# whwu95/MVFNet

Measured on AMD Instinct MI355X. Metric: clips/sec (fwd+bwd) MVFNet-R50 8x8 224^2, higher is better.
Workload: dtype bf16; 1 GPU; MVFNet-ResNet50 8x8, 32 clips/GPU of 8x3x224x224, bf16, train step: fwd (batch-stat BN) + loss + bwd + clip + SGD-nesterov; all through the HIP C ABI (stem + 16 bottlenecks + MVF + TSN head); clips_per_gpu=32, frames_per_clip=8, parallelism=dp1: replicas, one flat gradient all-reduce per step

## Files before the change

### mvfnet_amd/csrc/bn_dzfree.hip

```cpp
#include "common.h"

namespace {

typedef float f32x16 __attribute__((ext_vector_type(16)));
typedef short bf16x8 __attribute__((ext_vector_type(8)));

struct PrepArgs {
    const uint16_t* wd;
    const float *gamma, *mean, *invstd, *dgamma, *dbeta;
    uint16_t* bd;
    float* bias;
    int C, K;
    float inv_m;
    int g_wgs, s_wgs;
};

__device__ __forceinline__ float bf16lo(unsigned u) { return __uint_as_float(u << 16); }
__device__ __forceinline__ float bf16hi(unsigned u) { return __uint_as_float(u & 0xffff0000u); }

__global__ __launch_bounds__(256) void dzfree_prep_kernel(PrepArgs p) {
    extern __shared__ __attribute__((aligned(16))) float coef[];
    const int C = p.C, K = p.K, tid = threadIdx.x;
    float* ca = coef;
    float* ce = coef + C;
    float* ct = coef + 2 * C;
    for (int c = tid; c < C; c += 256) {
        const float r = p.invstd[c], a = p.gamma[c] * r, d0 = p.dbeta[c] * p.inv_m, kx = r * p.dgamma[c] * p.inv_m;
        ca[c] = a;
        ce[c] = a * kx;
        ct[c] = a * (d0 - kx * p.mean[c]);
    }
    __syncthreads();
    const int lane = tid & 63, wave = tid >> 6;
    int b = blockIdx.x;
    if (b < p.g_wgs) {
        const int kb = K / 32;
        const int j0 = (b / kb) * 32, k0 = (b % kb) * 32;
        const int row = lane & 31, half = lane >> 5;
        const int cq = C / 4, cbeg = wave * cq;
        const uint16_t* pa = p.wd + (long)(j0 + row) * C + half * 8;
        const uint16_t* pb = p.wd + (long)(k0 + row) * C + half * 8;
        f32x16 acc;
#pragma unroll
        for (int r = 0; r < 16; ++r) acc[r] = 0.f;
        uint4 va[4], vb[4], na[4], nb[4];
#pragma unroll
        for (int s_ = 0; s_ < 4; ++s_) {
            va[s_] = *reinterpret_cast<const uint4*>(pa + cbeg + s_ * 16);
            vb[s_] = *reinterpret_cast<const uint4*>(pb + cbeg + s_ * 16);
        }
        for (int c0 = cbeg; c0 < cbeg + cq; c0 += 64) {
            const bool more = c0 + 64 < cbeg + cq;
#pragma unroll
            for (int s_ = 0; s_ < 4; ++s_) {
                na[s_] = more ? *reinterpret_cast<const uint4*>(pa + c0 + 64 + s_ * 16) : make_uint4(0, 0, 0, 0);
                nb[s_] = more ? *reinterpret_cast<const uint4*>(pb + c0 + 64 + s_ * 16) : make_uint4(0, 0, 0, 0);
            }
#pragma unroll
            for (int s_ = 0; s_ < 4; ++s_) {
                const float4 e0 = *reinterpret_cast<const float4*>(ce + c0 + s_ * 16 + half * 8), e1 = *reinterpret_cast<const float4*>(ce + c0 + s_ * 16 + half * 8 + 4);
                uint4 sa;
                sa.x = pack_bf16x2(bf16lo(va[s_].x) * e0.x, bf16hi(va[s_].x) * e0.y);
                sa.y = pack_bf16x2(bf16lo(va[s_].y) * e0.z, bf16hi(va[s_].y) * e0.w);
                sa.z = pack_bf16x2(bf16lo(va[s_].z) * e1.x, bf16hi(va[s_].z) * e1.y);
                sa.w = pack_bf16x2(bf16lo(va[s_].w) * e1.z, bf16hi(va[s_].w) * e1.w);
                bf16x8 fa, fb;
                __builtin_memcpy(&fa, &sa, 16);
                __builtin_memcpy(&fb, &vb[s_], 16);
                acc = __builtin_amdgcn_mfma_f32_32x32x16_bf16(fa, fb, acc, 0, 0, 0);
            }
#pragma unroll
            for (int s_ = 0; s_ < 4; ++s_) { va[s_] = na[s_]; vb[s_] = nb[s_]; }
        }
        float* red = coef + 3 * C;
#pragma unroll
        for (int r = 0; r < 16; ++r) red[(wave * 16 + r) * 64 + lane] = acc[r];
        __syncthreads();
        float v[4];
#pragma unroll
        for (int i = 0; i < 4; ++i) v[i] = (red[(0 * 16 + 4 * wave + i) * 64 + lane] + red[(1 * 16 + 4 * wave + i) * 64 + lane]) +
                                           (red[(2 * 16 + 4 * wave + i) * 64 + lane] + red[(3 * 16 + 4 * wave + i) * 64 + lane]);
        uint2 pk;
        pk.x = pack_bf16x2(-v[0], -v[1]);
        pk.y = pack_bf16x2(-v[2], -v[3]);
        *reinterpret_cast<uint2*>(p.bd + (long)(k0 + row) * (C + K) + C + j0 + 4 * half + 8 * wave) = pk;
        return;
    }
    b -= p.g_wgs;
    if (b < p.s_wgs) {
        const long u = (long)b * 256 + tid, per_row = C / 8;
        if (u >= (long)K * per_row) return;
        const int k = (int)(u / per_row), c = (int)(u - (long)k * per_row) * 8;
        const uint4 v = *reinterpret_cast<const uint4*>(p.wd + (long)k * C + c);
        const float4 a0 = *reinterpret_cast<const float4*>(ca + c), a1 = *reinterpret_cast<const float4*>(ca + c + 4);
        uint4 o;
        o.x = pack_bf16x2(bf16lo(v.x) * a0.x, bf16hi(v.x) * a0.y);
        o.y = pack_bf16x2(bf16lo(v.y) * a0.z, bf16hi(v.y) * a0.w);
        o.z = pack_bf16x2(bf16lo(v.z) * a1.x, bf16hi(v.z) * a1.y);
        o.w = pack_bf16x2(bf16lo(v.w) * a1.z, bf16hi(v.w) * a1.w);
        *reinterpret_cast<uint4*>(p.bd + (long)k * (C + K) + c) = o;
        return;
    }
    b -= p.s_wgs;
    {
        const int k = b * 4 + wave;
        if (k >= K) return;
        float s = 0.f;
        for (int c = lane * 8; c < C; c += 512) {
            const uint4 v = *reinterpret_cast<const uint4*>(p.wd + (long)k * C + c);
            const float4 t0 = *reinterpret_cast<const float4*>(ct + c), t1 = *reinterpret_cast<const float4*>(ct + c + 4);
            s += bf16lo(v.x) * t0.x + bf16hi(v.x) * t0.y + bf16lo(v.y) * t0.z + bf16hi(v.y) * t0.w;
            s += bf16lo(v.z) * t1.x + bf16hi(v.z) * t1.y + bf16lo(v.w) * t1.z + bf16hi(v.w) * t1.w;
        }
        for (int off = 32; off >= 1; off >>= 1) s += __shfl_xor(s, off, 64);
        if (lane == 0) p.bias[k] = -s;
    }
}

__global__ __launch_bounds__(256) void dzfree_wgrad_fix_kernel(float* dw, const uint16_t* w, const float* gram, const float* a_mean, const float* gamma,
                                                               const float* mean, const float* invstd, const float* dgamma, const float* dbeta, int C, int K,
                                                               float m_f) {
    const int lane = threadIdx.x & 63, wave = threadIdx.x >> 6;
    const int kb = K / 32, blk = blockIdx.x * 4 + wave;
    if (blk >= (C / 32) * kb) return;
    const int c0 = (blk / kb) * 32, k0 = (blk % kb) * 32;
    const int row = lane & 31, half = lane >> 5;
    const uint16_t* pw = w + (long)(c0 + row) * K + half * 8;
    const float* pg = gram + (long)(k0 + row) * K + half * 8;
    f32x16 acc;
#pragma unroll
    for (int r = 0; r < 16; ++r) acc[r] = 0.f;
    constexpr int U = 4;
    for (int j = 0; j < K; j += 16 * U) {
        uint4 vw[U];
        float4 g0[U], g1[U];
#pragma unroll
        for (int u = 0; u < U; ++u) {
            vw[u] = *reinterpret_cast<const uint4*>(pw + j + 16 * u);
            g0[u] = *reinterpret_cast<const float4*>(pg + j + 16 * u);
            g1[u] = *reinterpret_cast<const float4*>(pg + j + 16 * u + 4);
        }
#pragma unroll
        for (int u = 0; u < U; ++u) {
            uint4 hi, lo;
            hi.x = pack_bf16x2(g0[u].x, g0[u].y); hi.y = pack_bf16x2(g0[u].z, g0[u].w);
            hi.z = pack_bf16x2(g1[u].x, g1[u].y); hi.w = pack_bf16x2(g1[u].z, g1[u].w);
            lo.x = pack_bf16x2(g0[u].x - bf16lo(hi.x), g0[u].y - bf16hi(hi.x)); lo.y = pack_bf16x2(g0[u].z - bf16lo(hi.y), g0[u].w - bf16hi(hi.y));
            lo.z = pack_bf16x2(g1[u].x - bf16lo(hi.z), g1[u].y - bf16hi(hi.z)); lo.w = pack_bf16x2(g1[u].z - bf16lo(hi.w), g1[u].w - bf16hi(hi.w));
            bf16x8 fw, fh, fl;
            __builtin_memcpy(&fw, &vw[u], 16);
            __builtin_memcpy(&fh, &hi, 16);
            __builtin_memcpy(&fl, &lo, 16);
            acc = __builtin_amdgcn_mfma_f32_32x32x16_bf16(fw, fh, acc, 0, 0, 0);
            acc = __builtin_amdgcn_mfma_f32_32x32x16_bf16(fw, fl, acc, 0, 0, 0);
        }
    }
    const float inv_m = 1.0f / m_f;
    const int k = k0 + row;
    const float sa = a_mean[k] * m_f;
#pragma unroll
    for (int r = 0; r < 16; ++r) {
        const int c = c0 + 8 * (r >> 2) + 4 * half + (r & 3);
        const float rs = invstd[c], a = gamma[c] * rs, d0 = dbeta[c] * inv_m, kx = rs * dgamma[c] * inv_m;
        const long i = (long)c * K + k;
        dw[i] = a * (dw[i] - d0 * sa - kx * (acc[r] - mean[c] * sa));
    }
}

__global__ __launch_bounds__(256) void dzfree_sums_kernel(const float* q, const uint16_t* w, int C, int K, const float* mean,
                                                          const float* invstd, const float* part_lo, int rows_lo, int c_split, const float* part_hi, int rows_hi,
                                                          float* dgamma, float* dbeta) {
    const int lane = threadIdx.x & 63, c = blockIdx.x * 4 + (threadIdx.x >> 6);
    if (c >= C) return;
    const bool lo = c < c_split;
    const int rows = lo ? rows_lo : rows_hi;
    const float2* p = reinterpret_cast<const float2*>(lo ? part_lo : part_hi) + (long)c * rows;
    float s1 = 0.f, dot = 0.f;
    for (int r = lane; r < rows; r += 64) s1 += p[r].x;
    const uint16_t* pw = w + (long)c * K;
    const float* pq = q + (long)c * K;
    for (int k = lane * 4; k < K; k += 256) {
        const uint2 wv = *reinterpret_cast<const uint2*>(pw + k);
        const float4 qv = *reinterpret_cast<const float4*>(pq + k);
        dot += bf16lo(wv.x) * qv.x + bf16hi(wv.x) * qv.y + bf16lo(wv.y) * qv.z + bf16hi(wv.y) * qv.w;
    }
#pragma unroll
    for (int o = 32; o > 0; o >>= 1) {
        s1 += __shfl_xor(s1, o, 64);
        dot += __shfl_xor(dot, o, 64);
    }
    if (lane == 0) {
        dbeta[c] = s1;
        dgamma[c] = invstd[c] * (dot - mean[c] * s1);
    }
}

struct GramStatsArgs {
    const float* gram; const float* a_mean; const uint16_t* w; const float* gamma; const float* beta;
    float* running_mean; float* running_var; float* save_mean; float* save_invstd; float* scale; float* shift;
    int C, K; float inv_m, eps, momentum, unbias;
};
__global__ __launch_bounds__(256) void gram_stats_kernel(GramStatsArgs p) {
    const int lane = threadIdx.x & 63, wave = threadIdx.x >> 6, K = p.K;
    const int blk = blockIdx.x * 4 + wave;
    if (blk >= p.C / 32) return;
    const int c0 = blk * 32, row = lane & 31, half = lane >> 5;
    const uint16_t* pw = p.w + (long)(c0 + row) * K + half * 8;
    float qacc[16], macc[16];
#pragma unroll
    for (int r = 0; r < 16; ++r) qacc[r] = macc[r] = 0.f;
    for (int kb = 0; kb < K / 32; ++kb) {
        const int k = kb * 32 + row;
        const float* pg = p.gram + (long)k * K + half * 8;
        const float* pa = p.a_mean + half * 8;
        const float ak = p.a_mean[k];
        f32x16 acc;
#pragma unroll
        for (int r = 0; r < 16; ++r) acc[r] = 0.f;
        for (int j = 0; j < K; j += 16) {
            const uint4 vw = *reinterpret_cast<const uint4*>(pw + j);
            const float4 g0 = *reinterpret_cast<const float4*>(pg + j), g1 = *reinterpret_cast<const float4*>(pg + j + 4);
            const float4 a0 = *reinterpret_cast<const float4*>(pa + j), a1 = *reinterpret_cast<const float4*>(pa + j + 4);
            float gc[8] = {g0.x * p.inv_m - ak * a0.x, g0.y * p.inv_m - ak * a0.y, g0.z * p.inv_m - ak * a0.z, g0.w * p.inv_m - ak * a0.w,
                           g1.x * p.inv_m - ak * a1.x, g1.y * p.inv_m - ak * a1.y, g1.z * p.inv_m - ak * a1.z, g1.w * p.inv_m - ak * a1.w};
            unsigned hi[4], mid[4], lo[4];
#pragma unroll
            for (int q = 0; q < 4; ++q) {
                const float x0 = gc[2 * q], x1 = gc[2 * q + 1];
                hi[q] = pack_bf16x2(x0, x1);
                const float r0 = x0 - bf16lo(hi[q]), r1 = x1 - bf16hi(hi[q]);
                mid[q] = pack_bf16x2(r0, r1);
                lo[q] = pack_bf16x2(r0 - bf16lo(mid[q]), r1 - bf16hi(mid[q]));
            }
            bf16x8 fw, fh, fm, fl;
            __builtin_memcpy(&fw, &vw, 16);
            __builtin_memcpy(&fh, hi, 16);
            __builtin_memcpy(&fm, mid, 16);
            __builtin_memcpy(&fl, lo, 16);
            acc = __builtin_amdgcn_mfma_f32_32x32x16_bf16(fw, fh, acc, 0, 0, 0);
            acc = __builtin_amdgcn_mfma_f32_32x32x16_bf16(fw, fm, acc, 0, 0, 0);
            acc = __builtin_amdgcn_mfma_f32_32x32x16_bf16(fw, fl, acc, 0, 0, 0);
        }
#pragma unroll
        for (int r = 0; r < 16; ++r) {
            const int c = c0 + 8 * (r >> 2) + 4 * half + (r & 3);
            const float wv = __uint_as_float((unsigned)p.w[(long)c * K + k] << 16);
            qacc[r] += acc[r] * wv;
            macc[r] += wv * ak;
        }
    }
#pragma unroll
    for (int r = 0; r < 16; ++r) {
#pragma unroll
        for (int o = 1; o < 32; o <<= 1) {
            qacc[r] += __shfl_xor(qacc[r], o, 64);
            macc[r] += __shfl_xor(macc[r], o, 64);
        }
    }
    if (row == 0) {
#pragma unroll
        for (int r = 0; r < 16; ++r) {
            const int c = c0 + 8 * (r >> 2) + 4 * half + (r & 3);
            const float mean = macc[r], var = fmaxf(qacc[r], 0.f);
            const float invstd = 1.0f / sqrtf(var + p.eps);
            p.save_mean[c] = mean;
            p.save_invstd[c] = invstd;
            const float s = p.gamma[c] * invstd;
            p.scale[c] = s;
            p.shift[c] = p.beta[c] - mean * s;
            if (p.running_mean) p.running_mean[c] = (1.f - p.momentum) * p.running_mean[c] + p.momentum * mean;
            if (p.running_var) p.running_var[c] = (1.f - p.momentum) * p.running_var[c] + p.momentum * (var * p.unbias);
        }
    }
}

}

extern "C" {

int mvf_bn_train_stats_gram(const float* gram, const float* a_mean, const void* w_packed, long m, int c, int k, const float* gamma, const float* beta, float eps,
                            float momentum, float* running_mean, float* running_var, float* save_mean, float* save_invstd, float* scale, float* shift,
                            int dtype, void* stream) {
    MVF_REQUIRE(gram && a_mean && w_packed && gamma && beta && save_mean && save_invstd && scale && shift && m > 0, MVF_EINVAL, "bn_train_stats_gram: NULL argument");
    MVF_REQUIRE(dtype == MVF_BF16, MVF_EUNSUPPORTED, "bn_train_stats_gram: bf16 storage only");
    MVF_REQUIRE(c > 0 && k > 0 && c % 32 == 0 && k % 32 == 0, MVF_ESHAPE, "bn_train_stats_gram: c=%d and k=%d must be multiples of 32", c, k);
    MVF_REQUIRE(((uintptr_t)gram | (uintptr_t)a_mean | (uintptr_t)w_packed) % 16 == 0, MVF_EINVAL, "bn_train_stats_gram: operands must be 16-byte aligned");
    GramStatsArgs p = {gram, a_mean, (const uint16_t*)w_packed, gamma, beta, running_mean, running_var, save_mean, save_invstd, scale, shift,
                       c, k, 1.0f / (float)m, eps, momentum, (float)((double)m / (double)(m > 1 ? m - 1 : 1))};
    hipLaunchKernelGGL(gram_stats_kernel, dim3((c / 32 + 3) / 4), dim3(256), 0, (hipStream_t)stream, p);
    MVF_LAUNCH_CHECK();
    return MVF_OK;
}

int mvf_bn_bwd_dzfree_sums(const float* q, const void* w_packed, int c, int k, const float* mean, const float* invstd,
                           const float* part_lo, int rows_lo, int c_split, const float* part_hi, int rows_hi, float* dgamma, float* dbeta, int dtype, void* stream) {
    MVF_REQUIRE(q && w_packed && mean && invstd && dgamma && dbeta, MVF_EINVAL, "bn_bwd_dzfree_sums: NULL argument");
    MVF_REQUIRE(dtype == MVF_BF16, MVF_EUNSUPPORTED, "bn_bwd_dzfree_sums: bf16 storage only");
    MVF_REQUIRE(c > 0 && k > 0 && k % 4 == 0 && c_split >= 0 && c_split <= c, MVF_ESHAPE, "bn_bwd_dzfree_sums: c=%d, k=%d (a multiple of 4), 0 <= c_split=%d <= c", c, k, c_split);
    MVF_REQUIRE((c_split == 0 || (part_lo && rows_lo > 0)) && (c_split == c || (part_hi && rows_hi > 0)), MVF_EINVAL, "bn_bwd_dzfree_sums: a channel range without partial sums");
    MVF_REQUIRE(((uintptr_t)q % 16 == 0) && ((uintptr_t)w_packed % 8 == 0), MVF_EINVAL, "bn_bwd_dzfree_sums: q must be 16-byte, w_packed 8-byte aligned");
    hipLaunchKernelGGL(dzfree_sums_kernel, dim3((c + 3) / 4), dim3(256), 0, (hipStream_t)stream, q, (const uint16_t*)w_packed, c, k, mean, invstd, part_lo, rows_lo,
                       c_split, part_hi, rows_hi, dgamma, dbeta);
    MVF_LAUNCH_CHECK();
    return MVF_OK;
}

int mvf_bn_bwd_dzfree_prep(const void* w_packed_dgrad, int c, int k, const float* gamma, const float* mean, const float* invstd, const float* dgamma,
                           const float* dbeta, long m, void* w_out, float* bias_out, int dtype, void* stream) {
    MVF_REQUIRE(w_packed_dgrad && gamma && mean && invstd && dgamma && dbeta && w_out && bias_out && m > 0, MVF_EINVAL, "bn_bwd_dzfree_prep: NULL argument");
    MVF_REQUIRE(dtype == MVF_BF16, MVF_EUNSUPPORTED, "bn_bwd_dzfree_prep: bf16 storage only");
    MVF_REQUIRE(c > 0 && k > 0 && c % 64 == 0 && k % 32 == 0 && c <= 4096, MVF_ESHAPE, "bn_bwd_dzfree_prep: c=%d must be a multiple of 64 (<= 4096), k=%d a multiple of 32", c, k);
    MVF_REQUIRE(((uintptr_t)w_packed_dgrad | (uintptr_t)w_out) % 16 == 0, MVF_EINVAL, "bn_bwd_dzfree_prep: operands must be 16-byte aligned");
    PrepArgs p = {};
    p.wd = (const uint16_t*)w_packed_dgrad; p.gamma = gamma; p.mean = mean; p.invstd = invstd; p.dgamma = dgamma; p.dbeta = dbeta;
    p.bd = (uint16_t*)w_out; p.bias = bias_out; p.C = c; p.K = k; p.inv_m = 1.0f / (float)m;
    MVF_REQUIRE(c % 256 == 0, MVF_ESHAPE, "bn_bwd_dzfree_prep: c=%d must be a multiple of 256 (four waves x 64-channel trips)", c);
    const int kb = k / 32;
    p.g_wgs = kb * kb;
    p.s_wgs = (int)(((long)k * (c / 8) + 255) / 256);
    const int b_wgs = (k + 3) / 4;
    const size_t lds = (size_t)3 * c * sizeof(float) + 4 * 16 * 64 * sizeof(float);
    hipLaunchKernelGGL(dzfree_prep_kernel, dim3(p.g_wgs + p.s_wgs + b_wgs), dim3(256), lds, (hipStream_t)stream, p);
    MVF_LAUNCH_CHECK();
    return MVF_OK;
}

int mvf_bn_bwd_dzfree_wgrad(float* dw, const void* w_packed, const float* gram, const float* a_mean, const float* gamma, const float* mean,
                            const float* invstd, const float* dgamma, const float* dbeta, long m, int c, int k, int dtype, void* stream) {
    MVF_REQUIRE(dw && w_packed && gram && a_mean && gamma && mean && invstd && dgamma && dbeta && m > 0, MVF_EINVAL, "bn_bwd_dzfree_wgrad: NULL argument");
    MVF_REQUIRE(dtype == MVF_BF16, MVF_EUNSUPPORTED, "bn_bwd_dzfree_wgrad: bf16 storage only");
    MVF_REQUIRE(c > 0 && c % 32 == 0 && k > 0 && k % 64 == 0, MVF_ESHAPE, "bn_bwd_dzfree_wgrad: c=%d must be a multiple of 32, k=%d of 64", c, k);
    MVF_REQUIRE(((uintptr_t)w_packed | (uintptr_t)gram) % 16 == 0, MVF_EINVAL, "bn_bwd_dzfree_wgrad: w_packed / gram must be 16-byte aligned");
    const int blocks = (c / 32) * (k / 32);
    hipLaunchKernelGGL(dzfree_wgrad_fix_kernel, dim3((blocks + 3) / 4), dim3(256), 0, (hipStream_t)stream, dw, (const uint16_t*)w_packed, gram, a_mean, gamma, mean,
                       invstd, dgamma, dbeta, c, k, (float)m);
    MVF_LAUNCH_CHECK();
    return MVF_OK;
}

}
```

### mvfnet_amd/csrc/pw_bwd_fused.hip

```cpp
#include <algorithm>
#include <type_traits>

#include "common.h"

namespace {

typedef float f32x16 __attribute__((ext_vector_type(16)));
typedef short bf16x8_t __attribute__((ext_vector_type(8)));
typedef unsigned u32x4 __attribute__((ext_vector_type(4)));

constexpr int kT = 512;
constexpr int CH = 64;
constexpr int NC = 256, NK = 64;
constexpr int PD = NC * 2;
constexpr int PX = NK * 2;
constexpr int PB = NC / 4;
constexpr unsigned kOOB = 0x80000000u;
constexpr int kOffD = 0, kOffX = CH * PD, kOffG = kOffX + 2 * CH * PX, kOffZ = kOffG + 2 * CH * PD, kOffM = kOffZ + 2 * CH * PX, kOffT = kOffM + 2 * CH * PB,
              kOffC = kOffT + CH * PX, kOffB = kOffC + 4 * NK * 4, kLds = kOffB + 4 * NC * 4;
static_assert(CH * 8 * 16 * 4 <= CH * PD, "the final reduction of the sums reuses a g buffer");
static_assert(kLds <= 160 * 1024, "LDS");

__device__ __forceinline__ int swz_d(int row) { return ((row & 3) << 2) | ((row >> 2) & 3); }
__device__ __forceinline__ int swz_x(int row) { return (((row >> 1) & 1) << 2) | ((row >> 2) & 3); }

__device__ __forceinline__ void unpack8(const u32x4 r, float (&f)[8]) {
    f[0] = __uint_as_float(r.x << 16); f[1] = __uint_as_float(r.x & 0xffff0000u);
    f[2] = __uint_as_float(r.y << 16); f[3] = __uint_as_float(r.y & 0xffff0000u);
    f[4] = __uint_as_float(r.z << 16); f[5] = __uint_as_float(r.z & 0xffff0000u);
    f[6] = __uint_as_float(r.w << 16); f[7] = __uint_as_float(r.w & 0xffff0000u);
}
__device__ __forceinline__ u32x4 pack8(const float (&f)[8]) {
    u32x4 r;
    r.x = pack_bf16x2(f[0], f[1]); r.y = pack_bf16x2(f[2], f[3]); r.z = pack_bf16x2(f[4], f[5]); r.w = pack_bf16x2(f[6], f[7]);
    return r;
}
__device__ __forceinline__ u32x4 lds16(const char* p) {
    const uint4 v = *reinterpret_cast<const uint4*>(p);
    u32x4 r;
    r.x = v.x; r.y = v.y; r.z = v.z; r.w = v.w;
    return r;
}
__device__ __forceinline__ void ldp8(const float* p, int c, float (&f)[8]) {
#pragma unroll
    for (int j = 0; j < 8; j += 4) {
        const float4 v = *reinterpret_cast<const float4*>(p + c + j);
        f[j] = v.x; f[j + 1] = v.y; f[j + 2] = v.z; f[j + 3] = v.w;
    }
}
__device__ __forceinline__ void lds_barrier() { asm volatile("s_waitcnt lgkmcnt(0)\n\ts_barrier" ::: "memory"); }
__device__ __forceinline__ void full_barrier() { asm volatile("s_waitcnt vmcnt(0) lgkmcnt(0)\n\ts_barrier" ::: "memory"); }
__device__ __forceinline__ void g_ahead_barrier() { asm volatile("s_waitcnt vmcnt(4) lgkmcnt(0)\n\ts_barrier" ::: "memory"); }

#ifdef policy pwbf_ablate
#define PWBF_ON(bit) if (!(a.ablate & (bit)))
#else
#define PWBF_ON(bit)
#endif

__global__ __launch_bounds__(kT) void pw_bwd_fused_kernel(const mvf_internal::PwBwdFusedArgs a) {
    extern __shared__ __attribute__((aligned(16))) char smem[];
    char* Ds = smem + kOffD;
    char* Xs = smem + kOffX;
    char* Gs = smem + kOffG;
    char* Zs = smem + kOffZ;
    char* Ms = smem + kOffM;
    char* Ts = smem + kOffT;
    float* Cs = reinterpret_cast<float*>(smem + kOffC);
    float* Bs = reinterpret_cast<float*>(smem + kOffB);

    const int split = blockIdx.x;
    const int m_begin = split * a.rows_per_split, m_end = min(a.M, m_begin + a.rows_per_split);
    const int nchunks = (m_end - m_begin + CH - 1) / CH;
    const int tid = threadIdx.x, lane = tid & 63, wave = __builtin_amdgcn_readfirstlane(tid >> 6);
    const int l31 = lane & 31, half = lane >> 5;
    const bool role_a = wave < 4;
    const bool sums = a.z_in != nullptr;

    const int q = tid & 31, r0 = tid >> 5;
    if (tid < NC) {
        const float inv_m = 1.0f / (float)a.M;
        const float rs = a.invstd[tid];
        Bs[tid] = a.gamma[tid] * rs; Bs[NC + tid] = a.dbeta[tid] * inv_m; Bs[2 * NC + tid] = rs * a.dgamma[tid] * inv_m; Bs[3 * NC + tid] = a.mean[tid];
    }
    if (sums && tid < NK) {
        Cs[tid] = a.in_scale[tid]; Cs[NK + tid] = a.in_shift[tid]; Cs[2 * NK + tid] = a.in_mean[tid]; Cs[3 * NK + tid] = a.in_invstd[tid];
    }

    const int pb3 = wave & 1, kb3 = (wave >> 1) & 1;
    bf16x8_t w1[4];
    {
        const char* wp = reinterpret_cast<const char*>(a.w);
#pragma unroll
        for (int ks = 0; ks < 4; ++ks) {
            const uint4 v = *reinterpret_cast<const uint4*>(wp + ((long)(32 * wave + l31) * NK + ks * 16 + half * 8) * 2);
            __builtin_memcpy(&w1[ks], &v, 16);
        }
    }

    const __amdgpu_buffer_rsrc_t rs_dx = __builtin_amdgcn_make_buffer_rsrc(a.dx, 0, (unsigned)min((long)a.M * NK * 2, 0x7ffffff0L), 0x00020000);

    const int rbx = tid >> 3;
    const int qbx = (tid & 7) ^ swz_x(rbx);
    const i32x4 gs_x = rsrc_words(a.a, (unsigned)min((long)a.M * a.aps * 2, 0x7ffffff0L));
    const i32x4 gs_g = rsrc_words(a.g, (unsigned)min((long)a.M * a.g_pitch * 2, 0x7ffffff0L));
    const i32x4 gs_z = rsrc_words(a.z_in, (unsigned)min((long)a.M * NK * 2, 0x7ffffff0L));
    const i32x4 gs_m = rsrc_words(a.bits, (unsigned)min((long)a.M * PB, 0x7ffffff0L));
// ... 150 lines not shown
#pragma unroll
                    for (int i = 0; i < 2; ++i) fa[i] = gather(Ds + ks * 16 * PD + offA[i][0], Ds + ks * 16 * PD + offA[i][1]);
#pragma unroll
                    for (int i = 0; i < 2; ++i)
#pragma unroll
                        for (int j = 0; j < 2; ++j) accw[i * 2 + j] = __builtin_amdgcn_mfma_f32_32x32x16_bf16(fa[i], fb[j], accw[i * 2 + j], 0, 0, 0);
                }
            }
        };
        auto gemm3 = [&]() {
            if constexpr (A) {
                const int row = pb3 * 32 + l31;
                int vx = half ^ swz_d(row);
                asm volatile("" : "+v"(vx));
                f32x16 acc;
#pragma unroll
                for (int r = 0; r < 16; ++r) acc[r] = 0.f;
#pragma unroll
                for (int ks = 0; ks < 16; ++ks) {
                    const u32x4 v = lds16(Ds + row * PD + (((ks * 2) ^ vx) * 16));
                    bf16x8_t bv;
                    __builtin_memcpy(&bv, &v, 16);
                    acc = __builtin_amdgcn_mfma_f32_32x32x16_bf16(wt[ks], bv, acc, 0, 0, 0);
                    if ((ks & 3) == 3) __builtin_amdgcn_sched_barrier(0);
                }
#pragma unroll
                for (int g4 = 0; g4 < 4; ++g4) {
                    uint2 pk;
                    pk.x = pack_bf16x2(acc[4 * g4], acc[4 * g4 + 1]);
                    pk.y = pack_bf16x2(acc[4 * g4 + 2], acc[4 * g4 + 3]);
                    *reinterpret_cast<uint2*>(Ts + row * PX + (((kb3 * 4 + g4) ^ swz_x(row)) * 16) + half * 8) = pk;
                }
            }
        };
        if (nchunks > 0) {
            dma_x(0);
            dma_mz(0);
            dma_g(0);
            if (nchunks > 1) dma_g(1);
        }
        full_barrier();
        for (int cc = 0; cc < nchunks; ++cc) {
            if (cc + 1 < nchunks) dma_x(cc + 1);
            PWBF_ON(32) finish(cc - 1);
            PWBF_ON(2) gemm1(cc & 1);
            lds_barrier();
            if (cc + 1 < nchunks) dma_mz(cc + 1);
            PWBF_ON(1) form_dz(cc & 1);
            lds_barrier();
            const bool g2 = cc + 2 < nchunks;
            PWBF_ON(16) if (g2) dma_g(cc + 2);
            PWBF_ON(8) gemm3();
            PWBF_ON(4) gemm2(cc & 1);
#ifdef policy pwbf_ablate
            full_barrier();
#else
            if (g2) g_ahead_barrier(); else full_barrier();
#endif
        }
        finish(nchunks - 1);
        if constexpr (!A) {
            float* out = a.part + (long)split * NC * NK;
            const int lr = lane >> 5, lc = lane & 31;
#pragma unroll
            for (int j = 0; j < 2; ++j) {
                const int col = j * 32 + lc;
#pragma unroll
                for (int i = 0; i < 2; ++i)
#pragma unroll
                    for (int r = 0; r < 16; ++r) {
                        const int row = (wq * 2 + i) * 32 + (r & 3) + 8 * (r >> 2) + 4 * lr;
                        out[(long)row * NK + col] = accw[i * 2 + j][r];
                    }
            }
        }
    };
    if (role_a) run(std::true_type());
    else run(std::false_type());

    __syncthreads();
    if (sums) {
        float* red = reinterpret_cast<float*>(Gs);
        float* dst = red + (re * 8 + ue) * 16;
        *reinterpret_cast<float4*>(dst) = make_float4(s1[0], s1[1], s1[2], s1[3]);
        *reinterpret_cast<float4*>(dst + 4) = make_float4(s1[4], s1[5], s1[6], s1[7]);
        *reinterpret_cast<float4*>(dst + 8) = make_float4(s2[0], s2[1], s2[2], s2[3]);
        *reinterpret_cast<float4*>(dst + 12) = make_float4(s2[4], s2[5], s2[6], s2[7]);
        __syncthreads();
        if (tid < NK) {
            const int u = tid >> 3, j = tid & 7;
            double t1 = 0.0, t2 = 0.0;
            for (int r = 0; r < CH; ++r) {
                t1 += (double)red[(r * 8 + u) * 16 + j];
                t2 += (double)red[(r * 8 + u) * 16 + 8 + j];
            }
            float2* p = reinterpret_cast<float2*>(a.sums_part) + (long)tid * a.sums_rows;
            const float h1 = (float)t1, h2 = (float)t2;
            p[split] = make_float2(h1, h2);
            p[a.nsplit + split] = make_float2((float)(t1 - (double)h1), (float)(t2 - (double)h2));
        }
    }
}

}

namespace mvf_internal {

int pw_bwd_fused_plan(long m, int c, int k, int* rows_per_split) {
    if (c != NC || k != NK || m <= 0 || m * (long)NC * 2 >= 0x7ffffff0L) return 0;
    static const int wgs_env = std::max(1, mvf_policy_int("pwbf_wgs", 256));
    long rows = (m + wgs_env - 1) / wgs_env;
    rows = (rows + CH - 1) / CH * CH;
    if (rows < 2 * CH) rows = 2 * CH;
    if (rows_per_split) *rows_per_split = (int)rows;
    return (int)((m + rows - 1) / rows);
}

int pw_bwd_fused_launch(const PwBwdFusedArgs& a0, hipStream_t st) {
    auto k = pw_bwd_fused_kernel;
    static bool attr = false;
    if (!attr) {
        MVF_HIP_OK(hipFuncSetAttribute((const void*)k, hipFuncAttributeMaxDynamicSharedMemorySize, kLds));
        attr = true;
    }
    PwBwdFusedArgs a = a0;
#ifdef policy pwbf_ablate
    a.ablate = mvf_policy_int("pwbf_ablate", 0);
#endif
    hipLaunchKernelGGL(k, dim3(a.nsplit), dim3(kT), kLds, st, a);
    MVF_LAUNCH_CHECK();
    return MVF_OK;
}

}
```

Measured before the change: 1836 clips/s.

## Rework BN dz-free kernels: wave-count templates, LDS gram strip, split reductions

The dz-free prep kernel is templated on wave count, with each work-group branch computing only the coefficients it needs and the bias branch handling two rows per wave. The wgrad fix kernel stages the hi/lo bf16 split of a 32-row gram strip in LDS once and reuses it across several channel blocks, with prefetched weight loads. The sums kernel gains a vectorized, prefetched dot path and an unrolled double-precision partial-sum reduction. Gram stats now spreads kb×kb units across 4 or 8 waves and reduces through shared memory. The aim is more parallelism and less redundant work in small BN-backward kernels, at the cost of extra LDS, barriers and a new k<=1024 limit.

```diff
diff --git a/mvfnet_amd/csrc/bn_dzfree.hip b/mvfnet_amd/csrc/bn_dzfree.hip
--- a/mvfnet_amd/csrc/bn_dzfree.hip
+++ b/mvfnet_amd/csrc/bn_dzfree.hip
@@ -18,37 +18,35 @@
 __device__ __forceinline__ float bf16lo(unsigned u) { return __uint_as_float(u << 16); }
 __device__ __forceinline__ float bf16hi(unsigned u) { return __uint_as_float(u & 0xffff0000u); }
 
-__global__ __launch_bounds__(256) void dzfree_prep_kernel(PrepArgs p) {
+template <int NW>
+__global__ __launch_bounds__(NW * 64) void dzfree_prep_kernel(PrepArgs p) {
     extern __shared__ __attribute__((aligned(16))) float coef[];
+    constexpr int NT = NW * 64;
     const int C = p.C, K = p.K, tid = threadIdx.x;
-    float* ca = coef;
-    float* ce = coef + C;
-    float* ct = coef + 2 * C;
-    for (int c = tid; c < C; c += 256) {
-        const float r = p.invstd[c], a = p.gamma[c] * r, d0 = p.dbeta[c] * p.inv_m, kx = r * p.dgamma[c] * p.inv_m;
-        ca[c] = a;
-        ce[c] = a * kx;
-        ct[c] = a * (d0 - kx * p.mean[c]);
-    }
-    __syncthreads();
     const int lane = tid & 63, wave = tid >> 6;
     int b = blockIdx.x;
     if (b < p.g_wgs) {
         const int kb = K / 32;
         const int j0 = (b / kb) * 32, k0 = (b % kb) * 32;
         const int row = lane & 31, half = lane >> 5;
-        const int cq = C / 4, cbeg = wave * cq;
+        const int cq = C / NW, cbeg = wave * cq;
         const uint16_t* pa = p.wd + (long)(j0 + row) * C + half * 8;
         const uint16_t* pb = p.wd + (long)(k0 + row) * C + half * 8;
-        f32x16 acc;
-#pragma unroll
-        for (int r = 0; r < 16; ++r) acc[r] = 0.f;
         uint4 va[4], vb[4], na[4], nb[4];
 #pragma unroll
         for (int s_ = 0; s_ < 4; ++s_) {
             va[s_] = *reinterpret_cast<const uint4*>(pa + cbeg + s_ * 16);
             vb[s_] = *reinterpret_cast<const uint4*>(pb + cbeg + s_ * 16);
         }
+        float* ce = coef;
+        for (int c = tid; c < C; c += NT) {
+            const float r = p.invstd[c], a = p.gamma[c] * r, kx = r * p.dgamma[c] * p.inv_m;
+            ce[c] = a * kx;
+        }
+        __syncthreads();
+        f32x16 acc;
+#pragma unroll
+        for (int r = 0; r < 16; ++r) acc[r] = 0.f;
         for (int c0 = cbeg; c0 < cbeg + cq; c0 += 64) {
             const bool more = c0 + 64 < cbeg + cq;
 #pragma unroll
@@ -72,26 +70,47 @@
 #pragma unroll
             for (int s_ = 0; s_ < 4; ++s_) { va[s_] = na[s_]; vb[s_] = nb[s_]; }
         }
-        float* red = coef + 3 * C;
+        float* red = coef + C;
 #pragma unroll
         for (int r = 0; r < 16; ++r) red[(wave * 16 + r) * 64 + lane] = acc[r];
         __syncthreads();
-        float v[4];
-#pragma unroll
-        for (int i = 0; i < 4; ++i) v[i] = (red[(0 * 16 + 4 * wave + i) * 64 + lane] + red[(1 * 16 + 4 * wave + i) * 64 + lane]) +
-                                           (red[(2 * 16 + 4 * wave + i) * 64 + lane] + red[(3 * 16 + 4 * wave + i) * 64 + lane]);
-        uint2 pk;
-        pk.x = pack_bf16x2(-v[0], -v[1]);
-        pk.y = pack_bf16x2(-v[2], -v[3]);
-        *reinterpret_cast<uint2*>(p.bd + (long)(k0 + row) * (C + K) + C + j0 + 4 * half + 8 * wave) = pk;
+        constexpr int PER = 16 / NW;
+        const int r0 = wave * PER;
+        float v[PER];
+#pragma unroll
+        for (int i = 0; i < PER; ++i) {
+            float s = red[(r0 + i) * 64 + lane];
+#pragma unroll
+            for (int wv = 1; wv < NW; ++wv) s += red[(wv * 16 + r0 + i) * 64 + lane];
+            v[i] = s;
+        }
+        uint16_t* dst = p.bd + (long)(k0 + row) * (C + K) + C + j0 + 8 * (r0 >> 2) + 4 * half + (r0 & 3);
+        if constexpr (PER == 4) {
+            uint2 pk;
+            pk.x = pack_bf16x2(-v[0], -v[1]);
+            pk.y = pack_bf16x2(-v[2], -v[3]);
+            *reinterpret_cast<uint2*>(dst) = pk;
+        } else if constexpr (PER == 2) {
+            *reinterpret_cast<uint32_t*>(dst) = pack_bf16x2(-v[0], -v[1]);
+        } else {
+            *dst = f32_to_bf16(-v[0]);
+        }
         return;
     }
     b -= p.g_wgs;
     if (b < p.s_wgs) {
-        const long u = (long)b * 256 + tid, per_row = C / 8;
-        if (u >= (long)K * per_row) return;
-        const int k = (int)(u / per_row), c = (int)(u - (long)k * per_row) * 8;
-        const uint4 v = *reinterpret_cast<const uint4*>(p.wd + (long)k * C + c);
+        const long u = (long)b * NT + tid, per_row = C / 8, total = (long)K * per_row;
+        uint4 v = make_uint4(0, 0, 0, 0);
+        int k = 0, c = 0;
+        if (u < total) {
+            k = (int)(u / per_row);
+            c = (int)(u - (long)k * per_row) * 8;
+            v = *reinterpret_cast<const uint4*>(p.wd + (long)k * C + c);
+        }
+        float* ca = coef;
+        for (int cc = tid; cc < C; cc += NT) ca[cc] = p.gamma[cc] * p.invstd[cc];
+        __syncthreads();
+        if (u >= total) return;
         const float4 a0 = *reinterpret_cast<const float4*>(ca + c), a1 = *reinterpret_cast<const float4*>(ca + c + 4);
         uint4 o;
         o.x = pack_bf16x2(bf16lo(v.x) * a0.x, bf16hi(v.x) * a0.y);
@@ -103,95 +122,160 @@
     }
     b -= p.s_wgs;
     {
-        const int k = b * 4 + wave;
+        float* ct = coef;
+        for (int c = tid; c < C; c += NT) {
+            const float r = p.invstd[c], a = p.gamma[c] * r, d0 = p.dbeta[c] * p.inv_m, kx = r * p.dgamma[c] * p.inv_m;
+            ct[c] = a * (d0 - kx * p.mean[c]);
+        }
+        __syncthreads();
+        const int k = (b * NW + wave) * 2;
         if (k >= K) return;
-        float s = 0.f;
+        float s0 = 0.f, s1 = 0.f;
         for (int c = lane * 8; c < C; c += 512) {
-            const uint4 v = *reinterpret_cast<const uint4*>(p.wd + (long)k * C + c);
+            const uint4 v = *reinterpret_cast<const uint4*>(p.wd + (long)k * C + c), x = *reinterpret_cast<const uint4*>(p.wd + (long)(k + 1) * C + c);
             const float4 t0 = *reinterpret_cast<const float4*>(ct + c), t1 = *reinterpret_cast<const float4*>(ct + c + 4);
-            s += bf16lo(v.x) * t0.x + bf16hi(v.x) * t0.y + bf16lo(v.y) * t0.z + bf16hi(v.y) * t0.w;
-            s += bf16lo(v.z) * t1.x + bf16hi(v.z) * t1.y + bf16lo(v.w) * t1.z + bf16hi(v.w) * t1.w;
-        }
-        for (int off = 32; off >= 1; off >>= 1) s += __shfl_xor(s, off, 64);
-        if (lane == 0) p.bias[k] = -s;
+            s0 += bf16lo(v.x) * t0.x + bf16hi(v.x) * t0.y + bf16lo(v.y) * t0.z + bf16hi(v.y) * t0.w;
+            s0 += bf16lo(v.z) * t1.x + bf16hi(v.z) * t1.y + bf16lo(v.w) * t1.z + bf16hi(v.w) * t1.w;
+            s1 += bf16lo(x.x) * t0.x + bf16hi(x.x) * t0.y + bf16lo(x.y) * t0.z + bf16hi(x.y) * t0.w;
+            s1 += bf16lo(x.z) * t1.x + bf16hi(x.z) * t1.y + bf16lo(x.w) * t1.z + bf16hi(x.w) * t1.w;
+        }
+        for (int off = 32; off >= 1; off >>= 1) {
+            s0 += __shfl_xor(s0, off, 64);
+            s1 += __shfl_xor(s1, off, 64);
+        }
+        if (lane == 0) {
+            p.bias[k] = -s0;
+            p.bias[k + 1] = -s1;
+        }
     }
 }
 
 __global__ __launch_bounds__(256) void dzfree_wgrad_fix_kernel(float* dw, const uint16_t* w, const float* gram, const float* a_mean, const float* gamma,
                                                                const float* mean, const float* invstd, const float* dgamma, const float* dbeta, int C, int K,
-                                                               float m_f) {
-    const int lane = threadIdx.x & 63, wave = threadIdx.x >> 6;
-    const int kb = K / 32, blk = blockIdx.x * 4 + wave;
-    if (blk >= (C / 32) * kb) return;
-    const int c0 = (blk / kb) * 32, k0 = (blk % kb) * 32;
+                                                               float m_f, int cpw) {
+    extern __shared__ __attribute__((aligned(16))) uint16_t strip[];
+    const int tid = threadIdx.x, lane = tid & 63, wave = tid >> 6;
+    const int P = K + 8, k0 = blockIdx.x * 32;
+    uint16_t* sh = strip;
+    uint16_t* sl = strip + 32 * P;
+    const int per_row = K / 8;
+#pragma unroll 4
+    for (int u = tid; u < 32 * per_row; u += 256) {
+        const int rr = u / per_row, j = (u - rr * per_row) * 8;
+        const float* pg = gram + (long)(k0 + rr) * K + j;
+        const float4 g0 = *reinterpret_cast<const float4*>(pg), g1 = *reinterpret_cast<const float4*>(pg + 4);
+        uint4 hi, lo;
+        hi.x = pack_bf16x2(g0.x, g0.y); hi.y = pack_bf16x2(g0.z, g0.w);
+        hi.z = pack_bf16x2(g1.x, g1.y); hi.w = pack_bf16x2(g1.z, g1.w);
+        lo.x = pack_bf16x2(g0.x - bf16lo(hi.x), g0.y - bf16hi(hi.x)); lo.y = pack_bf16x2(g0.z - bf16lo(hi.y), g0.w - bf16hi(hi.y));
+        lo.z = pack_bf16x2(g1.x - bf16lo(hi.z), g1.y - bf16hi(hi.z)); lo.w = pack_bf16x2(g1.z - bf16lo(hi.w), g1.w - bf16hi(hi.w));
+        *reinterpret_cast<uint4*>(sh + rr * P + j) = hi;
+        *reinterpret_cast<uint4*>(sl + rr * P + j) = lo;
+    }
+    __syncthreads();
     const int row = lane & 31, half = lane >> 5;
-    const uint16_t* pw = w + (long)(c0 + row) * K + half * 8;
-    const float* pg = gram + (long)(k0 + row) * K + half * 8;
-    f32x16 acc;
-#pragma unroll
-    for (int r = 0; r < 16; ++r) acc[r] = 0.f;
-    constexpr int U = 4;
-    for (int j = 0; j < K; j += 16 * U) {
-        uint4 vw[U];
-        float4 g0[U], g1[U];
-#pragma unroll
-        for (int u = 0; u < U; ++u) {
-            vw[u] = *reinterpret_cast<const uint4*>(pw + j + 16 * u);
-            g0[u] = *reinterpret_cast<const float4*>(pg + j + 16 * u);
-            g1[u] = *reinterpret_cast<const float4*>(pg + j + 16 * u + 4);
-        }
-#pragma unroll
-        for (int u = 0; u < U; ++u) {
-            uint4 hi, lo;
-            hi.x = pack_bf16x2(g0[u].x, g0[u].y); hi.y = pack_bf16x2(g0[u].z, g0[u].w);
-            hi.z = pack_bf16x2(g1[u].x, g1[u].y); hi.w = pack_bf16x2(g1[u].z, g1[u].w);
-            lo.x = pack_bf16x2(g0[u].x - bf16lo(hi.x), g0[u].y - bf16hi(hi.x)); lo.y = pack_bf16x2(g0[u].z - bf16lo(hi.y), g0[u].w - bf16hi(hi.y));
-            lo.z = pack_bf16x2(g1[u].x - bf16lo(hi.z), g1[u].y - bf16hi(hi.z)); lo.w = pack_bf16x2(g1[u].z - bf16lo(hi.w), g1[u].w - bf16hi(hi.w));
-            bf16x8 fw, fh, fl;
-            __builtin_memcpy(&fw, &vw[u], 16);
-            __builtin_memcpy(&fh, &hi, 16);
-            __builtin_memcpy(&fl, &lo, 16);
-            acc = __builtin_amdgcn_mfma_f32_32x32x16_bf16(fw, fh, acc, 0, 0, 0);
-            acc = __builtin_amdgcn_mfma_f32_32x32x16_bf16(fw, fl, acc, 0, 0, 0);
-        }
-    }
+    const uint16_t* ph = sh + row * P + half * 8;
+    const uint16_t* pl = sl + row * P + half * 8;
+    const int cb_end = min(C / 32, ((int)blockIdx.y + 1) * cpw);
     const float inv_m = 1.0f / m_f;
     const int k = k0 + row;
     const float sa = a_mean[k] * m_f;
-#pragma unroll
-    for (int r = 0; r < 16; ++r) {
-        const int c = c0 + 8 * (r >> 2) + 4 * half + (r & 3);
-        const float rs = invstd[c], a = gamma[c] * rs, d0 = dbeta[c] * inv_m, kx = rs * dgamma[c] * inv_m;
-        const long i = (long)c * K + k;
-        dw[i] = a * (dw[i] - d0 * sa - kx * (acc[r] - mean[c] * sa));
-    }
-}
-
+    constexpr int U = 4;
+    for (int cb = blockIdx.y * cpw + wave; cb < cb_end; cb += 4) {
+        const int c0 = cb * 32;
+        const uint16_t* pw = w + (long)(c0 + row) * K + half * 8;
+        f32x16 acc0, acc1;
+#pragma unroll
+        for (int r = 0; r < 16; ++r) acc0[r] = acc1[r] = 0.f;
+        uint4 vw[U], nw[U];
+#pragma unroll
+        for (int u = 0; u < U; ++u) vw[u] = *reinterpret_cast<const uint4*>(pw + 16 * u);
+        for (int j = 0; j < K; j += 16 * U) {
+            const bool more = j + 16 * U < K;
+#pragma unroll
+            for (int u = 0; u < U; ++u) nw[u] = more ? *reinterpret_cast<const uint4*>(pw + j + 16 * U + 16 * u) : make_uint4(0, 0, 0, 0);
+#pragma unroll
+            for (int u = 0; u < U; ++u) {
+                bf16x8 fw;
+                __builtin_memcpy(&fw, &vw[u], 16);
+                const bf16x8 fh = *reinterpret_cast<const bf16x8*>(ph + j + 16 * u), fl = *reinterpret_cast<const bf16x8*>(pl + j + 16 * u);
+                acc0 = __builtin_amdgcn_mfma_f32_32x32x16_bf16(fw, fh, acc0, 0, 0, 0);
+                acc1 = __builtin_amdgcn_mfma_f32_32x32x16_bf16(fw, fl, acc1, 0, 0, 0);
+            }
+#pragma unroll
+            for (int u = 0; u < U; ++u) vw[u] = nw[u];
+        }
+#pragma unroll
+        for (int r = 0; r < 16; ++r) {
+            const int c = c0 + 8 * (r >> 2) + 4 * half + (r & 3);
+            const float rs = invstd[c], a = gamma[c] * rs, d0 = dbeta[c] * inv_m, kx = rs * dgamma[c] * inv_m;
+            const long i = (long)c * K + k;
+            dw[i] = a * (dw[i] - d0 * sa - kx * ((acc0[r] + acc1[r]) - mean[c] * sa));
+        }
+    }
+}
+
+template <bool V8>
 __global__ __launch_bounds__(256) void dzfree_sums_kernel(const float* q, const uint16_t* w, int C, int K, const float* mean,
                                                           const float* invstd, const float* part_lo, int rows_lo, int c_split, const float* part_hi, int rows_hi,
                                                           float* dgamma, float* dbeta) {
+    constexpr int U = 16;
     const int lane = threadIdx.x & 63, c = blockIdx.x * 4 + (threadIdx.x >> 6);
     if (c >= C) return;
     const bool lo = c < c_split;
     const int rows = lo ? rows_lo : rows_hi;
     const float2* p = reinterpret_cast<const float2*>(lo ? part_lo : part_hi) + (long)c * rows;
-    float s1 = 0.f, dot = 0.f;
-    for (int r = lane; r < rows; r += 64) s1 += p[r].x;
     const uint16_t* pw = w + (long)c * K;
     const float* pq = q + (long)c * K;
-    for (int k = lane * 4; k < K; k += 256) {
-        const uint2 wv = *reinterpret_cast<const uint2*>(pw + k);
-        const float4 qv = *reinterpret_cast<const float4*>(pq + k);
-        dot += bf16lo(wv.x) * qv.x + bf16hi(wv.x) * qv.y + bf16lo(wv.y) * qv.z + bf16hi(wv.y) * qv.w;
-    }
+    float dot = 0.f, dot1 = 0.f;
+    if constexpr (V8) {
+        uint4 wv = make_uint4(0, 0, 0, 0);
+        float4 q0 = make_float4(0.f, 0.f, 0.f, 0.f), q1 = q0;
+        int k = lane * 8;
+        if (k < K) {
+            wv = *reinterpret_cast<const uint4*>(pw + k);
+            q0 = *reinterpret_cast<const float4*>(pq + k);
+            q1 = *reinterpret_cast<const float4*>(pq + k + 4);
+        }
+        for (; k < K; k += 512) {
+            uint4 nv = make_uint4(0, 0, 0, 0);
+            float4 n0 = make_float4(0.f, 0.f, 0.f, 0.f), n1 = n0;
+            if (k + 512 < K) {
+                nv = *reinterpret_cast<const uint4*>(pw + k + 512);
+                n0 = *reinterpret_cast<const float4*>(pq + k + 512);
+                n1 = *reinterpret_cast<const float4*>(pq + k + 516);
+            }
+            dot += bf16lo(wv.x) * q0.x + bf16hi(wv.x) * q0.y + bf16lo(wv.y) * q0.z + bf16hi(wv.y) * q0.w;
+            dot1 += bf16lo(wv.z) * q1.x + bf16hi(wv.z) * q1.y + bf16lo(wv.w) * q1.z + bf16hi(wv.w) * q1.w;
+            wv = nv; q0 = n0; q1 = n1;
+        }
+    }
+    double a0 = 0.0, a1 = 0.0;
+    for (int r = lane; r < rows; r += U * 64) {
+        float2 v[U];
+#pragma unroll
+        for (int u = 0; u < U; ++u) v[u] = r + u * 64 < rows ? p[r + u * 64] : make_float2(0.f, 0.f);
+#pragma unroll
+        for (int u = 0; u < U; u += 2) { a0 += (double)v[u].x; a1 += (double)v[u + 1].x; }
+    }
+    if constexpr (!V8) {
+        for (int k = lane * 4; k < K; k += 256) {
+            const uint2 wv = *reinterpret_cast<const uint2*>(pw + k);
+            const float4 qv = *reinterpret_cast<const float4*>(pq + k);
+            dot += bf16lo(wv.x) * qv.x + bf16hi(wv.x) * qv.y + bf16lo(wv.y) * qv.z + bf16hi(wv.y) * qv.w;
+        }
+    }
+    double s1 = a0 + a1;
+    dot += dot1;
 #pragma unroll
     for (int o = 32; o > 0; o >>= 1) {
         s1 += __shfl_xor(s1, o, 64);
         dot += __shfl_xor(dot, o, 64);
     }
     if (lane == 0) {
-        dbeta[c] = s1;
-        dgamma[c] = invstd[c] * (dot - mean[c] * s1);
+        const float s = (float)s1;
+        dbeta[c] = s;
+        dgamma[c] = invstd[c] * (dot - mean[c] * s);
     }
 }
 
@@ -200,27 +284,44 @@
     float* running_mean; float* running_var; float* save_mean; float* save_invstd; float* scale; float* shift;
     int C, K; float inv_m, eps, momentum, unbias;
 };
-__global__ __launch_bounds__(256) void gram_stats_kernel(GramStatsArgs p) {
-    const int lane = threadIdx.x & 63, wave = threadIdx.x >> 6, K = p.K;
-    const int blk = blockIdx.x * 4 + wave;
-    if (blk >= p.C / 32) return;
-    const int c0 = blk * 32, row = lane & 31, half = lane >> 5;
+template <int NW>
+__global__ __launch_bounds__(NW * 64) void gram_stats_kernel(GramStatsArgs p) {
+    __shared__ float red[NW][2][32];
+    const int tid = threadIdx.x, lane = tid & 63, wave = tid >> 6, K = p.K;
+    const int c0 = blockIdx.x * 32, row = lane & 31, half = lane >> 5;
+    const int kbs = K / 32, units = kbs * kbs;
     const uint16_t* pw = p.w + (long)(c0 + row) * K + half * 8;
     float qacc[16], macc[16];
 #pragma unroll
     for (int r = 0; r < 16; ++r) qacc[r] = macc[r] = 0.f;
-    for (int kb = 0; kb < K / 32; ++kb) {
+    for (int un = wave; un < units; un += NW) {
+        const int kb = un / kbs, j0 = (un - kb * kbs) * 32;
         const int k = kb * 32 + row;
-        const float* pg = p.gram + (long)k * K + half * 8;
-        const float* pa = p.a_mean + half * 8;
+        const float* pg = p.gram + (long)k * K + j0 + half * 8;
+        const float* pa = p.a_mean + j0 + half * 8;
         const float ak = p.a_mean[k];
-        f32x16 acc;
-#pragma unroll
-        for (int r = 0; r < 16; ++r) acc[r] = 0.f;
-        for (int j = 0; j < K; j += 16) {
-            const uint4 vw = *reinterpret_cast<const uint4*>(pw + j);
-            const float4 g0 = *reinterpret_cast<const float4*>(pg + j), g1 = *reinterpret_cast<const float4*>(pg + j + 4);
-            const float4 a0 = *reinterpret_cast<const float4*>(pa + j), a1 = *reinterpret_cast<const float4*>(pa + j + 4);
+        uint4 vw[2];
+        float4 g[2][2], am[2][2];
+        unsigned wv2[8];
+#pragma unroll
+        for (int t = 0; t < 2; ++t) {
+            vw[t] = *reinterpret_cast<const uint4*>(pw + j0 + 16 * t);
+            g[t][0] = *reinterpret_cast<const float4*>(pg + 16 * t);
+            g[t][1] = *reinterpret_cast<const float4*>(pg + 16 * t + 4);
+            am[t][0] = *reinterpret_cast<const float4*>(pa + 16 * t);
+            am[t][1] = *reinterpret_cast<const float4*>(pa + 16 * t + 4);
+        }
+#pragma unroll
+        for (int r = 0; r < 16; r += 2) {
+            const int c = c0 + 8 * (r >> 2) + 4 * half + (r & 3);
+            wv2[r >> 1] = (unsigned)p.w[(long)c * K + k] | ((unsigned)p.w[(long)(c + 1) * K + k] << 16);
+        }
+        f32x16 acc[2];
+#pragma unroll
+        for (int t = 0; t < 2; ++t) {
+#pragma unroll
+            for (int r = 0; r < 16; ++r) acc[t][r] = 0.f;
+            const float4 g0 = g[t][0], g1 = g[t][1], a0 = am[t][0], a1 = am[t][1];
             float gc[8] = {g0.x * p.inv_m - ak * a0.x, g0.y * p.inv_m - ak * a0.y, g0.z * p.inv_m - ak * a0.z, g0.w * p.inv_m - ak * a0.w,
                            g1.x * p.inv_m - ak * a1.x, g1.y * p.inv_m - ak * a1.y, g1.z * p.inv_m - ak * a1.z, g1.w * p.inv_m - ak * a1.w};
             unsigned hi[4], mid[4], lo[4];
@@ -233,20 +334,19 @@
                 lo[q] = pack_bf16x2(r0 - bf16lo(mid[q]), r1 - bf16hi(mid[q]));
             }
             bf16x8 fw, fh, fm, fl;
-            __builtin_memcpy(&fw, &vw, 16);
+            __builtin_memcpy(&fw, &vw[t], 16);
             __builtin_memcpy(&fh, hi, 16);
             __builtin_memcpy(&fm, mid, 16);
             __builtin_memcpy(&fl, lo, 16);
-            acc = __builtin_amdgcn_mfma_f32_32x32x16_bf16(fw, fh, acc, 0, 0, 0);
-            acc = __builtin_amdgcn_mfma_f32_32x32x16_bf16(fw, fm, acc, 0, 0, 0);
-            acc = __builtin_amdgcn_mfma_f32_32x32x16_bf16(fw, fl, acc, 0, 0, 0);
+            acc[t] = __builtin_amdgcn_mfma_f32_32x32x16_bf16(fw, fh, acc[t], 0, 0, 0);
+            acc[t] = __builtin_amdgcn_mfma_f32_32x32x16_bf16(fw, fm, acc[t], 0, 0, 0);
+            acc[t] = __builtin_amdgcn_mfma_f32_32x32x16_bf16(fw, fl, acc[t], 0, 0, 0);
         }
 #pragma unroll
         for (int r = 0; r < 16; ++r) {
-            const int c = c0 + 8 * (r >> 2) + 4 * half + (r & 3);
-            const float wv = __uint_as_float((unsigned)p.w[(long)c * K + k] << 16);
-            qacc[r] += acc[r] * wv;
-            macc[r] += wv * ak;
+            const float wv = (r & 1) ? bf16hi(wv2[r >> 1]) : bf16lo(wv2[r >> 1]);
+            qacc[r] += (acc[0][r] + acc[1][r]) * wv;
+            if (j0 == 0) macc[r] += wv * ak;
         }
     }
 #pragma unroll
@@ -260,18 +360,46 @@
     if (row == 0) {
 #pragma unroll
         for (int r = 0; r < 16; ++r) {
-            const int c = c0 + 8 * (r >> 2) + 4 * half + (r & 3);
-            const float mean = macc[r], var = fmaxf(qacc[r], 0.f);
-            const float invstd = 1.0f / sqrtf(var + p.eps);
-            p.save_mean[c] = mean;
-            p.save_invstd[c] = invstd;
-            const float s = p.gamma[c] * invstd;
-            p.scale[c] = s;
-            p.shift[c] = p.beta[c] - mean * s;
-            if (p.running_mean) p.running_mean[c] = (1.f - p.momentum) * p.running_mean[c] + p.momentum * mean;
-            if (p.running_var) p.running_var[c] = (1.f - p.momentum) * p.running_var[c] + p.momentum * (var * p.unbias);
-        }
-    }
+            red[wave][0][8 * (r >> 2) + 4 * half + (r & 3)] = qacc[r];
+            red[wave][1][8 * (r >> 2) + 4 * half + (r & 3)] = macc[r];
+        }
+    }
+    __syncthreads();
+    if (tid < 32) {
+        float qs = red[0][0][tid], ms = red[0][1][tid];
+#pragma unroll
+        for (int wv = 1; wv < NW; ++wv) {
+            qs += red[wv][0][tid];
+            ms += red[wv][1][tid];
+        }
+        const int c = c0 + tid;
+        const float mean = ms, var = fmaxf(qs, 0.f);
+        const float invstd = 1.0f / sqrtf(var + p.eps);
+        p.save_mean[c] = mean;
+        p.save_invstd[c] = invstd;
+        const float s = p.gamma[c] * invstd;
+        p.scale[c] = s;
+        p.shift[c] = p.beta[c] - mean * s;
+        if (p.running_mean) p.running_mean[c] = (1.f - p.momentum) * p.running_mean[c] + p.momentum * mean;
+        if (p.running_var) p.running_var[c] = (1.f - p.momentum) * p.running_var[c] + p.momentum * (var * p.unbias);
+    }
+}
+
+template <int NW>
+int launch_prep(PrepArgs p, hipStream_t st) {
+    const int kb = p.K / 32;
+    p.g_wgs = kb * kb;
+    p.s_wgs = (int)(((long)p.K * (p.C / 8) + NW * 64 - 1) / (NW * 64));
+    const int b_wgs = (p.K + 2 * NW - 1) / (2 * NW);
+    const size_t lds = ((size_t)p.C + (size_t)NW * 16 * 64) * sizeof(float);
+    static bool attr = false;
+    if (!attr) {
+        MVF_HIP_OK(hipFuncSetAttribute((const void*)dzfree_prep_kernel<NW>, hipFuncAttributeMaxDynamicSharedMemorySize, (4096 + NW * 16 * 64) * (int)sizeof(float)));
+        attr = true;
+    }
+    hipLaunchKernelGGL(dzfree_prep_kernel<NW>, dim3(p.g_wgs + p.s_wgs + b_wgs), dim3(NW * 64), lds, st, p);
+    MVF_LAUNCH_CHECK();
+    return MVF_OK;
 }
 
 }
@@ -287,7 +415,10 @@
     MVF_REQUIRE(((uintptr_t)gram | (uintptr_t)a_mean | (uintptr_t)w_packed) % 16 == 0, MVF_EINVAL, "bn_train_stats_gram: operands must be 16-byte aligned");
     GramStatsArgs p = {gram, a_mean, (const uint16_t*)w_packed, gamma, beta, running_mean, running_var, save_mean, save_invstd, scale, shift,
                        c, k, 1.0f / (float)m, eps, momentum, (float)((double)m / (double)(m > 1 ? m - 1 : 1))};
-    hipLaunchKernelGGL(gram_stats_kernel, dim3((c / 32 + 3) / 4), dim3(256), 0, (hipStream_t)stream, p);
+    if ((k / 32) * (k / 32) <= 4)
+        hipLaunchKernelGGL(gram_stats_kernel<4>, dim3(c / 32), dim3(256), 0, (hipStream_t)stream, p);
+    else
+        hipLaunchKernelGGL(gram_stats_kernel<8>, dim3(c / 32), dim3(512), 0, (hipStream_t)stream, p);
     MVF_LAUNCH_CHECK();
     return MVF_OK;
 }
@@ -299,8 +430,12 @@
     MVF_REQUIRE(c > 0 && k > 0 && k % 4 == 0 && c_split >= 0 && c_split <= c, MVF_ESHAPE, "bn_bwd_dzfree_sums: c=%d, k=%d (a multiple of 4), 0 <= c_split=%d <= c", c, k, c_split);
     MVF_REQUIRE((c_split == 0 || (part_lo && rows_lo > 0)) && (c_split == c || (part_hi && rows_hi > 0)), MVF_EINVAL, "bn_bwd_dzfree_sums: a channel range without partial sums");
     MVF_REQUIRE(((uintptr_t)q % 16 == 0) && ((uintptr_t)w_packed % 8 == 0), MVF_EINVAL, "bn_bwd_dzfree_sums: q must be 16-byte, w_packed 8-byte aligned");
-    hipLaunchKernelGGL(dzfree_sums_kernel, dim3((c + 3) / 4), dim3(256), 0, (hipStream_t)stream, q, (const uint16_t*)w_packed, c, k, mean, invstd, part_lo, rows_lo,
-                       c_split, part_hi, rows_hi, dgamma, dbeta);
+    if (k % 8 == 0 && (uintptr_t)w_packed % 16 == 0)
+        hipLaunchKernelGGL(dzfree_sums_kernel<true>, dim3((c + 3) / 4), dim3(256), 0, (hipStream_t)stream, q, (const uint16_t*)w_packed, c, k, mean, invstd, part_lo,
+                           rows_lo, c_split, part_hi, rows_hi, dgamma, dbeta);
+    else
+        hipLaunchKernelGGL(dzfree_sums_kernel<false>, dim3((c + 3) / 4), dim3(256), 0, (hipStream_t)stream, q, (const uint16_t*)w_packed, c, k, mean, invstd, part_lo,
+                           rows_lo, c_split, part_hi, rows_hi, dgamma, dbeta);
     MVF_LAUNCH_CHECK();
     return MVF_OK;
 }
@@ -315,25 +450,27 @@
     p.wd = (const uint16_t*)w_packed_dgrad; p.gamma = gamma; p.mean = mean; p.invstd = invstd; p.dgamma = dgamma; p.dbeta = dbeta;
     p.bd = (uint16_t*)w_out; p.bias = bias_out; p.C = c; p.K = k; p.inv_m = 1.0f / (float)m;
     MVF_REQUIRE(c % 256 == 0, MVF_ESHAPE, "bn_bwd_dzfree_prep: c=%d must be a multiple of 256 (four waves x 64-channel trips)", c);
-    const int kb = k / 32;
-    p.g_wgs = kb * kb;
-    p.s_wgs = (int)(((long)k * (c / 8) + 255) / 256);
-    const int b_wgs = (k + 3) / 4;
-    const size_t lds = (size_t)3 * c * sizeof(float) + 4 * 16 * 64 * sizeof(float);
-    hipLaunchKernelGGL(dzfree_prep_kernel, dim3(p.g_wgs + p.s_wgs + b_wgs), dim3(256), lds, (hipStream_t)stream, p);
-    MVF_LAUNCH_CHECK();
-    return MVF_OK;
+    if (c % 1024 == 0) return launch_prep<16>(p, (hipStream_t)stream);
+    if (c % 512 == 0) return launch_prep<8>(p, (hipStream_t)stream);
+    return launch_prep<4>(p, (hipStream_t)stream);
 }
 
 int mvf_bn_bwd_dzfree_wgrad(float* dw, const void* w_packed, const float* gram, const float* a_mean, const float* gamma, const float* mean,
                             const float* invstd, const float* dgamma, const float* dbeta, long m, int c, int k, int dtype, void* stream) {
     MVF_REQUIRE(dw && w_packed && gram && a_mean && gamma && mean && invstd && dgamma && dbeta && m > 0, MVF_EINVAL, "bn_bwd_dzfree_wgrad: NULL argument");
     MVF_REQUIRE(dtype == MVF_BF16, MVF_EUNSUPPORTED, "bn_bwd_dzfree_wgrad: bf16 storage only");
-    MVF_REQUIRE(c > 0 && c % 32 == 0 && k > 0 && k % 64 == 0, MVF_ESHAPE, "bn_bwd_dzfree_wgrad: c=%d must be a multiple of 32, k=%d of 64", c, k);
+    MVF_REQUIRE(c > 0 && c % 32 == 0 && k > 0 && k % 64 == 0 && k <= 1024, MVF_ESHAPE, "bn_bwd_dzfree_wgrad: c=%d must be a multiple of 32, k=%d of 64 (<= 1024: the LDS strip)", c, k);
     MVF_REQUIRE(((uintptr_t)w_packed | (uintptr_t)gram) % 16 == 0, MVF_EINVAL, "bn_bwd_dzfree_wgrad: w_packed / gram must be 16-byte aligned");
-    const int blocks = (c / 32) * (k / 32);
-    hipLaunchKernelGGL(dzfree_wgrad_fix_kernel, dim3((blocks + 3) / 4), dim3(256), 0, (hipStream_t)stream, dw, (const uint16_t*)w_packed, gram, a_mean, gamma, mean,
-                       invstd, dgamma, dbeta, c, k, (float)m);
+    const int cbs = c / 32, kbs = k / 32;
+    const int cpw = 4 * (int)(((long)cbs * kbs + 1023) / 1024);
+    const size_t lds = (size_t)2 * 32 * (k + 8) * sizeof(uint16_t);
+    static bool attr = false;
+    if (!attr) {
+        MVF_HIP_OK(hipFuncSetAttribute((const void*)dzfree_wgrad_fix_kernel, hipFuncAttributeMaxDynamicSharedMemorySize, 2 * 32 * (1024 + 8) * (int)sizeof(uint16_t)));
+        attr = true;
+    }
+    hipLaunchKernelGGL(dzfree_wgrad_fix_kernel, dim3(kbs, (cbs + cpw - 1) / cpw), dim3(256), lds, (hipStream_t)stream, dw, (const uint16_t*)w_packed, gram, a_mean, gamma,
+                       mean, invstd, dgamma, dbeta, c, k, (float)m, cpw);
     MVF_LAUNCH_CHECK();
     return MVF_OK;
 }
diff --git a/mvfnet_amd/csrc/pw_bwd_fused.hip b/mvfnet_amd/csrc/pw_bwd_fused.hip
--- a/mvfnet_amd/csrc/pw_bwd_fused.hip
+++ b/mvfnet_amd/csrc/pw_bwd_fused.hip
@@ -52,7 +52,7 @@
 __device__ __forceinline__ void full_barrier() { asm volatile("s_waitcnt vmcnt(0) lgkmcnt(0)\n\ts_barrier" ::: "memory"); }
 __device__ __forceinline__ void g_ahead_barrier() { asm volatile("s_waitcnt vmcnt(4) lgkmcnt(0)\n\ts_barrier" ::: "memory"); }
 
-#ifdef policy pwbf_ablate
+#ifdef MVF_PWBF_ABLATE
 #define PWBF_ON(bit) if (!(a.ablate & (bit)))
 #else
 #define PWBF_ON(bit)
@@ -309,7 +309,7 @@
             PWBF_ON(16) if (g2) dma_g(cc + 2);
             PWBF_ON(8) gemm3();
             PWBF_ON(4) gemm2(cc & 1);
-#ifdef policy pwbf_ablate
+#ifdef MVF_PWBF_ABLATE
             full_barrier();
 #else
             if (g2) g_ahead_barrier(); else full_barrier();
@@ -381,7 +381,7 @@
         attr = true;
     }
     PwBwdFusedArgs a = a0;
-#ifdef policy pwbf_ablate
+#ifdef MVF_PWBF_ABLATE
     a.ablate = mvf_policy_int("pwbf_ablate", 0);
 #endif
     hipLaunchKernelGGL(k, dim3(a.nsplit), dim3(kT), kLds, st, a);
```

Result: no change. 1849 clips/s, median of 6 (+0.7%).
